# menezesandre/stackrl

Measured on AMD Instinct MI355X. Metric: env steps/sec (batched Stack-v0), higher is better.
Workload: dtype f32

## Files before the change

### stackrl_amd/csrc/settle.hip

```cpp
#include "srl_device.h"
#include "srl_kernels.h"
#include "stage.h"

#ifdef SRL_DIAG_JITTER
__device__ __forceinline__ void srl_jitter_sync() {
  unsigned t = (unsigned)__builtin_readcyclecounter() * 2654435761u + (threadIdx.x >> 6) * 40503u;
  t = __builtin_amdgcn_readfirstlane(t);
  const int n = (t >> 13) & 15;
  for (int i = 0; i < n; ++i) __builtin_amdgcn_s_sleep(16);
  __builtin_amdgcn_fence(__ATOMIC_RELEASE, "workgroup");
  __builtin_amdgcn_s_barrier();
  __builtin_amdgcn_fence(__ATOMIC_ACQUIRE, "workgroup");
  t = t * 1664525u + 1013904223u;
  const int m = (t >> 13) & 15;
  for (int i = 0; i < m; ++i) __builtin_amdgcn_s_sleep(16);
}
#define __syncthreads() srl_jitter_sync()
#endif

#ifndef SRL_GJK_GROUP
#define SRL_GJK_GROUP(T, PP) ((T) == 128 && (PP) == 1 ? 32 : 16)
#endif

__device__ __forceinline__ int pair_word(int p) {
  int j = (int)((1.0f + sqrtf(1.0f + 8.0f * (float)p)) * 0.5f);
  while (j * (j - 1) / 2 > p) --j;
  while ((j + 1) * j / 2 <= p) ++j;
  return (p - j * (j - 1) / 2) | (j << 16);
}

enum { M_MODE = 0, M_U, M_V, M_NEXT, M_ZMAX, M_FLAGS, M_NCOL, M_CNT, M_NB, M_PENDING, M_STATUS, M_DONE, M_ORIENT, M_MOVING, M_RES0, M_RES1, M_SOLO, M_WORDS = 20 };

struct Lds {
  float* sm;
  const DevParams* P;
  int oX, oQ, oV, oPX, oPQ, oMESH, oGM, oMAN, oSOP, oPOS, oCOL, oR, oIW, oAMIN, oAMAX, oBC, oWV, oLV, oMISC, oPAIR, vs3;
  __device__ __forceinline__ void init(float* sm_, const DevParams* P_) {
    sm = sm_; P = P_;
    oX = P->OFF_X; oQ = P->OFF_Q; oV = P->OFF_V; oPX = P->OFF_PX; oPQ = P->OFF_PQ; oMESH = P->OFF_MESH;
    oGM = P->OFF_GM; oMAN = P->OFF_MAN; oSOP = P->OFF_SOP; oPOS = P->OFF_POS; oCOL = P->OFF_COL;
    const int blob = P->BLOB;
    oR = blob + P->S_R; oIW = blob + P->S_IW; oAMIN = blob + P->S_AMIN; oAMAX = blob + P->S_AMAX; oBC = blob + P->S_BC;
    oWV = blob + P->S_WV; oLV = blob + P->S_LV; oMISC = blob + P->S_MISC; oPAIR = blob + P->S_PAIR; vs3 = 3 * P->VS;
#ifndef SRL_NO_LAUNDER
#define SRL_KEEP(x) asm volatile("" : "+s"(x))
    SRL_KEEP(oX); SRL_KEEP(oQ); SRL_KEEP(oV); SRL_KEEP(oPX); SRL_KEEP(oPQ); SRL_KEEP(oMESH); SRL_KEEP(oGM);
    SRL_KEEP(oMAN); SRL_KEEP(oSOP); SRL_KEEP(oPOS); SRL_KEEP(oCOL); SRL_KEEP(oR); SRL_KEEP(oIW); SRL_KEEP(oAMIN);
    SRL_KEEP(oAMAX); SRL_KEEP(oBC); SRL_KEEP(oWV); SRL_KEEP(oLV); SRL_KEEP(oMISC); SRL_KEEP(oPAIR); SRL_KEEP(vs3);
#undef SRL_KEEP
#endif
  }
  __device__ __forceinline__ float* X(int b) const { return sm + oX + 4 * b; }
  __device__ __forceinline__ float* Q(int b) const { return sm + oQ + 4 * b; }
  __device__ __forceinline__ float* VW(int b) const { return sm + oV + 8 * b; }
  __device__ __forceinline__ float* PX(int b) const { return sm + oPX + 4 * b; }
  __device__ __forceinline__ float* PQ(int b) const { return sm + oPQ + 4 * b; }
  __device__ __forceinline__ int* MESH() const { return (int*)(sm + oMESH); }
  __device__ __forceinline__ float* GM(int b) const { return sm + oGM + SRL_GM_WORDS * b; }
  __device__ __forceinline__ float* MAN(int s) const { return sm + oMAN + SRL_MAN_WORDS * s; }
  __device__ __forceinline__ int* SOP() const { return (int*)(sm + oSOP); }
  __device__ __forceinline__ int* POS() const { return (int*)(sm + oPOS); }
  __device__ __forceinline__ int* COL() const { return (int*)(sm + oCOL); }
  __device__ __forceinline__ float* R(int b) const { return sm + oR + 9 * b; }
  __device__ __forceinline__ float* IW(int b) const { return sm + oIW + 9 * b; }
  __device__ __forceinline__ float* AMIN(int b) const { return sm + oAMIN + 3 * b; }
  __device__ __forceinline__ float* AMAX(int b) const { return sm + oAMAX + 3 * b; }
  __device__ __forceinline__ float* BC(int b) const { return sm + oBC + 8 * b; }
  __device__ __forceinline__ float* WV(int b) const { return sm + oWV + vs3 * b; }
  __device__ __forceinline__ float* LV(int b) const { return sm + oLV + vs3 * b; }
  __device__ __forceinline__ int* MISC() const { return (int*)(sm + oMISC); }
  __device__ __forceinline__ int* PAIR() const { return (int*)(sm + oPAIR); }
  __device__ __forceinline__ void pair(int p, int& i, int& j) const { const int w = PAIR()[p]; i = w & 0xffff; j = w >> 16; }
};

typedef float f2 __attribute__((ext_vector_type(2)));
typedef float f4 __attribute__((ext_vector_type(4)));
__device__ __forceinline__ f2 F2(float a, float b) { f2 r; r.x = a; r.y = b; return r; }
__device__ __forceinline__ f2 fma2(f2 a, f2 b, f2 c) { return __builtin_elementwise_fma(a, b, c); }

__device__ __forceinline__ void ldvw(const Lds& L, int b, v3& v, v3& w) {
  const float4 a = *(const float4*)L.VW(b);
  const float2 c = *(const float2*)(L.VW(b) + 4);
  v = V(a.x, a.z, c.x); w = V(a.y, a.w, c.y);
}
__device__ __forceinline__ v3 ldv(const Lds& L, int b) { const float* p = L.VW(b); return V(p[0], p[2], p[4]); }
__device__ __forceinline__ void stvw(const Lds& L, int b, v3 v, v3 w) {
  *(float4*)L.VW(b) = make_float4(v.x, w.x, v.y, w.y);
  *(float2*)(L.VW(b) + 4) = make_float2(v.z, w.z);
}

__device__ void goal_from_rng(const DevParams& P, uint32_t key, uint32_t episode, int32_t* rect) {
  int H = P.c.overhead_res;
  uint32_t bbit = srl_rng(key, episode, SRL_STREAM_GOAL, 0) >> 31;
  uint32_t u0 = srl_rng(key, episode, SRL_STREAM_GOAL, 1) >> 8;
  uint32_t u1 = srl_rng(key, episode, SRL_STREAM_GOAL, 2) >> 8;
  uint32_t u2 = srl_rng(key, episode, SRL_STREAM_GOAL, 3) >> 8;
  uint32_t lo = u0 < u1 ? u0 : u1; lo = lo < u2 ? lo : u2;
  uint32_t hi = u0 > u1 ? u0 : u1; hi = hi > u2 ? hi : u2;
  uint32_t X = bbit ? hi : lo;
  int h = P.goal_min_h + (int)(((uint64_t)X * (uint64_t)(P.goal_max_h - P.goal_min_h)) >> 24);
  int w = P.goal_size / h;
  if (w < P.goal_min_w) w = P.goal_min_w;
  if (w > P.goal_max_w) w = P.goal_max_w;
  int umax = H - h, vmax = H - w;
  int ulo = umax / 8, uhi = 7 * umax / 8 + 1;
  int vlo = vmax / 8, vhi = 7 * vmax / 8 + 1;
  rect[0] = ulo + (int)srl_rng_below(srl_rng(key, episode, SRL_STREAM_GOAL, 4), (uint32_t)(uhi - ulo));
  rect[1] = vlo + (int)srl_rng_below(srl_rng(key, episode, SRL_STREAM_GOAL, 5), (uint32_t)(vhi - vlo));
  rect[2] = h; rect[3] = w;
}

__device__ void env_reset(const DevParams& P, EnvHdr* h, int e) {
  int L = P.c.episode_length;
  uint32_t key = P.seed + (uint32_t)P.c.env_index_offset + (uint32_t)e;
// ... 647 lines not shown
  if (WARM) {
    p.in = p.in * ws; p.i1 = p.i1 * ws; p.i2 = p.i2 * ws;
    prow_apply(p.n, u, p.in);
    prow_apply(p.t1, u, p.i1);
    prow_apply(p.t2, u, p.i2);
  } else {
    prow_solve(p.n, u, p.target, p.in, 0.0f, 1e30f, res);
    const float lim = p.mu * p.in;
    prow_solve(p.t1, u, 0.0f, p.i1, -lim, lim, res);
    prow_solve(p.t2, u, 0.0f, p.i2, -lim, lim, res);
  }
  *(float4*)pa = make_float4(u.a[0].x, u.a[0].y, u.a[1].x, u.a[1].y); *(float2*)(pa + 4) = make_float2(u.a[2].x, u.a[2].y);
  *(float4*)pb = make_float4(u.b[0].x, u.b[0].y, u.b[1].x, u.b[1].y); *(float2*)(pb + 4) = make_float2(u.b[2].x, u.b[2].y);
}

template <bool WARM, int PP, bool SOLO, bool GB, bool GA>
__device__ __forceinline__ bool solver_sweep(const Lds& L, GPoint& gp, GBody& gb, Point (&pp)[PP], int ncol, int gslot,
                                             const int (&pslot)[PP], int gsweep, const unsigned long long (&cm)[2]) {
  float res = 0.0f;
  constexpr unsigned long long T0 = 0x1111111111111111ull;
  if (!GB) {
    const unsigned long long gm = __ballot(gslot >= 0);
#pragma unroll
    for (int i = 0; i < SRL_GMAXP; ++i) {
      const unsigned long long t = gm & (T0 << i);
      if (t == 0) break;
      if (__builtin_amdgcn_inverse_ballot_w64(t)) ground_turn<WARM>(L, gp, res);
      __builtin_amdgcn_wave_barrier();
    }
  } else {
    if (gb.np > 0) ground_body<WARM, !WARM && GA>(L, gb, res);
    __builtin_amdgcn_wave_barrier();
  }
  int c0 = 0;
#ifndef SRL_NO_COLOUR_MASKS
  if (SOLO && PP == 1) {
#pragma unroll
    for (int c = 0; c < 2; ++c) {
      if (c >= ncol) break;
#pragma unroll
      for (int i = 0; i < 4; ++i) {
        const unsigned long long t = cm[c] & (T0 << i);
        if (t == 0) break;
        if (__builtin_amdgcn_inverse_ballot_w64(t)) point_turn<WARM>(L, pp[0], res);
        __builtin_amdgcn_wave_barrier();
      }
    }
    c0 = 2;
  }
#endif
#pragma unroll 1
  for (int c = c0; c < ncol; ++c) {
    if (!SOLO) __syncthreads();
    unsigned long long mc[PP];
#pragma unroll
    for (int r = 0; r < PP; ++r) mc[r] = __ballot((pslot[r] >> 2) == c);
#pragma unroll
    for (int i = 0; i < 4; ++i) {
      unsigned long long any = 0;
#pragma unroll
      for (int r = 0; r < PP; ++r) any |= mc[r] & (T0 << i);
      if (any == 0) break;
#pragma unroll
      for (int r = 0; r < PP; ++r)
        if (__builtin_amdgcn_inverse_ballot_w64(mc[r] & (T0 << i))) point_turn<WARM>(L, pp[r], res);
      __builtin_amdgcn_wave_barrier();
    }
  }
  if (SOLO) return WARM ? true : __ballot(res * res > L.P->c.residual_threshold) != 0ull;
  int* word = L.MISC() + M_RES0 + (gsweep & 1);
  if (!WARM) {
    if (__ballot(res * res > L.P->c.residual_threshold) != 0ull && (threadIdx.x & 63) == 0) *word = gsweep;
  }
  __syncthreads();
  return WARM ? true : *word == gsweep;
}

#ifdef SRL_STAMPS
#define STAMP(k) do { if (tid == 0) { long long _t = wall_clock64(); L.P->hdr[blockIdx.x].stamps[k] += _t - _t0; _t0 = _t; } } while (0)
#else
#define STAMP(k)
#endif

template <int T, int PP>
__device__ __forceinline__ void substep(const Lds& L, int nb, int tid, int& gsweep) {
  const DevParams& P = *L.P;
  if (PP >= 2) asm volatile("" : "+v"(tid));
#ifdef SRL_STAMPS
  long long _t0 = wall_clock64();
#endif
  int* misc = L.MISC();
  if (tid < nb) body_frame(L, tid);
  if (tid == 0) { misc[M_FLAGS] = 0; misc[M_SOLO] = 1; }
  __syncthreads();
  STAMP(0);
  for (int it = tid; it < nb * P.VS; it += T) {
    const int b = it / P.VS, k = it - b * P.VS;
    if (k < __float_as_int(L.BC(b)[5])) {
      const m3 R = ldm(L.R(b));
      v3 lv;
      if (P.S_LV >= 0) lv = ld3(L.LV(b) + 3 * k);
      else { const float4 g4 = P.mv[__float_as_int(L.BC(b)[6]) + k]; lv = V(g4.x, g4.y, g4.z); }
      st3(L.WV(b) + 3 * k, mmul_add(R, lv, ld3(L.X(b))));
    }
  }
  __syncthreads();
  STAMP(1);
  for (int b = tid >> 4; b < nb; b += T >> 4) body_bounds_ground(L, b, tid & 15);
  __syncthreads();
  STAMP(2);
  const int npair = nb * (nb - 1) / 2;
  int fl = 0;
  for (int pid = tid; pid < npair; pid += T) {
    int i, j; L.pair(pid, i, j);
    v3 ai = ld3(L.AMIN(i)), bi = ld3(L.AMAX(i)), aj = ld3(L.AMIN(j)), bj = ld3(L.AMAX(j));
    bool ov = ai.x <= bj.x && aj.x <= bi.x && ai.y <= bj.y && aj.y <= bi.y && ai.z <= bj.z && aj.z <= bi.z;
    int sl = L.SOP()[pid];
    if (!ov && sl >= 0) { L.SOP()[pid] = -1; L.POS()[sl] = -1; fl |= 1; }
    if (ov && sl < 0) fl |= 2;
  }
  if (fl) atomicOr(&misc[M_FLAGS], fl);
  __syncthreads();
  const int flags = misc[M_FLAGS], ncol0 = misc[M_NCOL];
  if (flags || ncol0 < 0) {
    __syncthreads();
    if (tid == 0) {
      if (flags & 2) {
        for (int pid = 0; pid < npair; ++pid) {
          if (L.SOP()[pid] >= 0) continue;
          int i, j; L.pair(pid, i, j);
          v3 ai = ld3(L.AMIN(i)), bi = ld3(L.AMAX(i)), aj = ld3(L.AMIN(j)), bj = ld3(L.AMAX(j));
          bool ov = ai.x <= bj.x && aj.x <= bi.x && ai.y <= bj.y && aj.y <= bi.y && ai.z <= bj.z && aj.z <= bi.z;
          if (!ov) continue;
          int sl = -1;
          for (int k = 0; k < P.NS; ++k) if (L.POS()[k] < 0) { sl = k; break; }
          if (sl < 0) { misc[M_STATUS] |= SRL_ST_PAIR_OVERFLOW; atomicOr(P.flags, 4); continue; }
          L.SOP()[pid] = sl; L.POS()[sl] = pid;
          float* mp = L.MAN(sl);
          mp[0] = __int_as_float(0);
          mp[56] = __int_as_float(0);
          st3(mp + 1, ld3(L.X(i)) - ld3(L.X(j)));
        }
      }
      uint64_t* used = (uint64_t*)(L.sm + P.BLOB + P.S_USED);
      for (int b = 0; b < SRL_MAX_BODIES; ++b) used[b] = 0;
      int nc = 0;
      for (int sl = 0; sl < P.NS; ++sl) {
        int pid = L.POS()[sl];
        if (pid < 0) continue;
        int i, j; L.pair(pid, i, j);
        uint64_t u = used[i] | used[j];
        int c = __ffsll((long long)~u) - 1;
        L.COL()[sl] = c;
        used[i] |= (uint64_t)1 << c;
        used[j] |= (uint64_t)1 << c;
        if (c + 1 > nc) nc = c + 1;
      }
      misc[M_NCOL] = nc;
    }
    __syncthreads();
  }
  const int ncol = misc[M_NCOL];
  STAMP(3);
  {
    constexpr int G = SRL_GJK_GROUP(T, PP);
    const int gl = tid & (G - 1);
    for (int sl = tid / G; sl < P.NS; sl += T / G)
      if (L.POS()[sl] >= 0) narrowphase_slot<G>(L, sl, gl);
  }
  __syncthreads();
  STAMP(4);
  {
    GPoint gp = make_ground_point(L, tid / SRL_GMAXP, tid % SRL_GMAXP);
    if (tid / SRL_GMAXP >= nb) gp.valid = false;
    Point pp[PP];
#pragma unroll
    for (int r = 0; r < PP; ++r) pp[r] = make_pair_point(L, (tid + r * T) >> 2, tid & 3);
    {
      bool mine = gp.valid;
#pragma unroll
      for (int r = 0; r < PP; ++r) mine |= pp[r].valid;
      if (tid >= 64 && __ballot(mine) != 0ull && (tid & 63) == 0) misc[M_SOLO] = 0;
    }
    __syncthreads();
    GBody gb;
    gb.np = 0; gb.b = 0; gb.ima = 0.0f;
    gb.pvw = L.VW(0); gb.rec = cg_rec(L, 0, 0);
#pragma unroll
    for (int i = 0; i < SRL_GMAXP; ++i) { gb.acc[i][0] = 0.0f; gb.acc[i][1] = 0.0f; gb.acc[i][2] = 0.0f; }
#ifdef SRL_GROUND_TURNS
    constexpr bool GB = false;
#else
    constexpr bool GB = !(T == 256 && PP == 1);
#endif
#ifndef SRL_GA_MASK
#define SRL_GA_MASK 1
#endif
    constexpr bool GA = GB && ((T == 128 && PP == 1 && (SRL_GA_MASK & 1)) || (T == 128 && PP == 2 && (SRL_GA_MASK & 2)) ||
                               (T == 256 && PP == 2 && (SRL_GA_MASK & 4)));
    if (GB) {
    if (gp.valid) cg_store(L, gp);
    if (tid < nb) {
      const float* g = L.GM(tid);
      gb.b = tid; gb.np = __float_as_int(g[0]); gb.ima = L.BC(tid)[0];
      gb.pvw = L.VW(tid); gb.rec = cg_rec(L, tid, 0);
#pragma unroll
      for (int i = 0; i < SRL_GMAXP; ++i)
        if (i < gb.np) { gb.acc[i][0] = g[SRL_GM_IN + i]; gb.acc[i][1] = g[SRL_GM_T1 + i]; gb.acc[i][2] = g[SRL_GM_T2 + i]; }
    }
    __syncthreads();
    }
    STAMP(5);
#ifdef SRL_DIAG_NOSOLO
    const bool solo = false;
#else
    const bool solo = PP == 1 && misc[M_SOLO] != 0;
#endif
    const int gslot = gp.valid ? gp.idx : -1;
    unsigned long long cm[2];
    cm[0] = __ballot(pp[0].valid && pp[0].colour == 0); cm[1] = __ballot(pp[0].valid && pp[0].colour == 1);
    int pslot[PP];
#pragma unroll
    for (int r = 0; r < PP; ++r) pslot[r] = pp[r].valid ? 4 * pp[r].colour + pp[r].idx : -1;
    if (solo) {
      int done = 0;
      if (tid < 64) {
        bool anyp = false;
#pragma unroll
        for (int r = 0; r < PP; ++r) anyp |= pp[r].valid;
#ifdef SRL_NO_GROUND_ONLY
        const bool ground_only = false;
#else
        const bool ground_only = GB && __ballot(anyp) == 0ull;
#endif
        if (ground_only) {
          v3 v = V(0.0f, 0.0f, 0.0f), w = V(0.0f, 0.0f, 0.0f);
          if (gb.np > 0) {
            const float4 a0 = *(const float4*)gb.pvw;
            const float2 a1 = *(const float2*)(gb.pvw + 4);
            v = V(a0.x, a0.z, a1.x); w = V(a0.y, a0.w, a1.y);
            float res = 0.0f;
            ground_body_keep<true, false>(L, gb, v, w, res);
          }
          for (int it = 0; it < P.c.solver_iterations; ++it) {
            done++;
            float res = 0.0f;
            if (gb.np > 0) ground_body_keep<false, GA>(L, gb, v, w, res);
            if (__ballot(res * res > P.c.residual_threshold) == 0ull) break;
          }
          if (gb.np > 0) { *(float4*)gb.pvw = make_float4(v.x, w.x, v.y, w.y); *(float2*)(gb.pvw + 4) = make_float2(v.z, w.z); }
        } else {
          solver_sweep<true, PP, PP == 1, GB, GA>(L, gp, gb, pp, ncol, gslot, pslot, 0, cm);
          for (int it = 0; it < P.c.solver_iterations; ++it) {
            done++;
            if (!solver_sweep<false, PP, PP == 1, GB, GA>(L, gp, gb, pp, ncol, gslot, pslot, 0, cm)) break;
          }
        }
        if (tid == 0) misc[M_CNT] = done;
      }
      __syncthreads();
      gsweep += misc[M_CNT];
    } else {
      solver_sweep<true, PP, false, GB, GA>(L, gp, gb, pp, ncol, gslot, pslot, 0, cm);
      for (int it = 0; it < P.c.solver_iterations; ++it) {
        gsweep++;
        if (!solver_sweep<false, PP, false, GB, GA>(L, gp, gb, pp, ncol, gslot, pslot, gsweep, cm)) break;
      }
    }
#ifdef SRL_STAMPS
    if (tid == 0) {
      EnvHdr* hh = &L.P->hdr[blockIdx.x];
      bool anyp = false;
      for (int r = 0; r < PP; ++r) anyp |= pp[r].valid;
      {
        int bl[SRL_MAX_BODIES]; for (int b = 0; b < SRL_MAX_BODIES; ++b) bl[b] = 0;
        int lmax = 0, sumt = 0;
        for (int c = 0; c < ncol; ++c) {
          int mx = 0;
          for (int sl = 0; sl < P.NS; ++sl) {
            const int pid = L.POS()[sl];
            if (pid < 0 || L.COL()[sl] != c) continue;
            const int np = __float_as_int(L.MAN(sl)[0]);
            if (np <= 0) continue;
            int a, b; L.pair(pid, a, b);
            const int st = bl[a] > bl[b] ? bl[a] : bl[b];
            bl[a] = st + np; bl[b] = st + np;
            if (st + np > lmax) lmax = st + np;
            if (np > mx) mx = np;
          }
          sumt += mx;
        }
        hh->diag[4] += sumt; hh->diag[5] += lmax;
      }
      hh->diag[0] += 1; hh->diag[1] += (__ballot(anyp) == 0ull); hh->diag[2] += ncol; hh->diag[3] += solo ? misc[M_CNT] : 0;
    }
#endif
    if (!GB) {
      if (gp.valid) { float* g = L.GM(gp.a); g[SRL_GM_IN + gp.idx] = gp.in; g[SRL_GM_T1 + gp.idx] = gp.i1; g[SRL_GM_T2 + gp.idx] = gp.i2; }
    } else if (gb.np > 0) {
      float* g = L.GM(gb.b);
#pragma unroll
      for (int i = 0; i < SRL_GMAXP; ++i)
        if (i < gb.np) { g[SRL_GM_IN + i] = gb.acc[i][0]; g[SRL_GM_T1 + i] = gb.acc[i][1]; g[SRL_GM_T2 + i] = gb.acc[i][2]; }
    }
#pragma unroll
    for (int r = 0; r < PP; ++r)
      if (pp[r].valid) {
        float* q = L.MAN((tid + r * T) >> 2) + 4 + SRL_MP_WORDS * pp[r].idx;
        q[10] = pp[r].in; q[11] = pp[r].i1; q[12] = pp[r].i2;
      }
  }
  STAMP(6);
  const float dt = P.c.sim_time_step;
  if (tid < nb) {
    const int b = tid;
    v3 v, w;
    ldvw(L, b, v, w);
    st3(L.X(b), madd(ld3(L.X(b)), v, dt));
    float* Q = L.Q(b);
    q4 q; q.x = Q[0]; q.y = Q[1]; q.z = Q[2]; q.w = Q[3];
    float hx = 0.5f * dt;
    q4 dq;
    dq.x = hx * ((w.x * q.w + w.y * q.z) - w.z * q.y);
    dq.y = hx * ((w.y * q.w + w.z * q.x) - w.x * q.z);
    dq.z = hx * ((w.z * q.w + w.x * q.y) - w.y * q.x);
    dq.w = hx * (-((w.x * q.x + w.y * q.y) + w.z * q.z));
    q.x += dq.x; q.y += dq.y; q.z += dq.z; q.w += dq.w;
    float inv = 1.0f / sqrtf((q.x * q.x + q.y * q.y) + (q.z * q.z + q.w * q.w));
    Q[0] = q.x * inv; Q[1] = q.y * inv; Q[2] = q.z * inv; Q[3] = q.w * inv;
  }
  __syncthreads();
  STAMP(7);
}

__device__ __forceinline__ bool sim_stop(const Lds& L, int nb, int tid) {
  int* misc = L.MISC();
  bool moving = false;
  if (tid < nb) {
    v3 v = ldv(L, tid);
    moving = sqrtf(dot(v, v)) > L.P->c.velocity_threshold;
  }
  if (tid < 64) {
    const unsigned long long m = __ballot(moving);
    if (tid == 0) misc[M_MOVING] = m != 0ull;
  }
  __syncthreads();
  const int any = misc[M_MOVING];
  __syncthreads();
  return !any;
}

__device__ __forceinline__ int newest_contacts(const Lds& L, int nb, int tid, int T) {
  int* misc = L.MISC();
  if (tid == 0) misc[M_CNT] = __float_as_int(L.GM(nb - 1)[0]);
  __syncthreads();
  int n = 0;
  for (int sl = tid; sl < L.P->NS; sl += T) {
    int pid = L.POS()[sl];
    int pi_ = -1, pj_ = -1;
    if (pid >= 0) L.pair(pid, pi_, pj_);
    if (pid >= 0 && (pi_ == nb - 1 || pj_ == nb - 1)) n += __float_as_int(L.MAN(sl)[0]);
  }
  if (n) atomicAdd(&misc[M_CNT], n);
  __syncthreads();
  int r = misc[M_CNT];
  __syncthreads();
  return r;
}

__device__ __forceinline__ MeshHdr stage_mesh_hdr(const MeshHdr* __restrict__ mh, int m) {
  MeshHdr r;
  r.vo = __builtin_amdgcn_readfirstlane(mh[m].vo); r.nv = __builtin_amdgcn_readfirstlane(mh[m].nv);
  r.to = __builtin_amdgcn_readfirstlane(mh[m].to); r.nt = __builtin_amdgcn_readfirstlane(mh[m].nt);
  r.eo = __builtin_amdgcn_readfirstlane(mh[m].eo); r.ne = __builtin_amdgcn_readfirstlane(mh[m].ne);
  r.inv_mass = 0.0f; r.iix = 0.0f; r.iiy = 0.0f; r.iiz = 0.0f; r.radius = 0.0f; r.cx = 0.0f; r.cy = 0.0f; r.cz = 0.0f;
  return r;
}

#ifdef SRL_STAGE_TAIL_INLINE
#define SRL_TAIL_ATTR __forceinline__
#else
#define SRL_TAIL_ATTR __attribute__((noinline))
#endif
template <int T>
__device__ SRL_TAIL_ATTR void stage_tail(const DevParams* __restrict__ Pp, float4* __restrict__ stage, int e, int nb) {
  const DevParams& P = *Pp;
  extern __shared__ __attribute__((aligned(16))) float sm[];
  const int tid = threadIdx.x;
  const int wave = __builtin_amdgcn_readfirstlane(tid >> 6), lane = tid & 63;
  StageLds& S = ((StageLds*)(sm + P.BLOB))[wave];
  StageArgs A;
  A.mp = P.mp; A.mt = P.mt; A.me = P.me; A.mv = P.mv; A.px = P.px; A.inv_px = P.inv_px; A.res = P.c.overhead_res;
  const int slots = P.c.episode_length;
  const float* X = sm + P.OFF_X;
  const float* Q = sm + P.OFF_Q;
  const int* MESH = (const int*)(sm + P.OFF_MESH);
  float4* rec0 = stage + (size_t)e * slots * SRL_STAGE_STRIDE;
  int b = wave;
  if (b >= nb) return;
  MeshHdr mh = stage_mesh_hdr(P.mh, __builtin_amdgcn_readfirstlane(MESH[b]));
  StageLoads g = stage_request(A, mh, lane);
  for (;;) {
    const int bn = b + T / 64;
    const bool more = bn < nb;
    MeshHdr mh_n = mh;
    StageLoads g_n = g;
    if (more) { mh_n = stage_mesh_hdr(P.mh, __builtin_amdgcn_readfirstlane(MESH[bn])); g_n = stage_request(A, mh_n, lane); }
    const float* qq = Q + 4 * b;
    q4 q; q.x = qq[0]; q.y = qq[1]; q.z = qq[2]; q.w = qq[3];
    stage_compute(A, S, rec0 + (size_t)b * SRL_STAGE_STRIDE, ld3(X + 4 * b), q, mh, g, lane);
    __builtin_amdgcn_wave_barrier();
    if (!more) break;
// ... 70 lines not shown
        misc[M_RES0] = -1; misc[M_RES1] = -1;
      }
    }
    h->mode = mode;
    misc[M_MODE] = mode;
  }
  __syncthreads();
  const int mode = misc[M_MODE];
  if (mode == 1) {
    int* gi = (int*)gblob;
    for (int k = tid; k < P.NP; k += T) gi[P.OFF_SOP + k] = -1;
    for (int k = tid; k < P.NS; k += T) gi[P.OFF_POS + k] = -1;
    return;
  }
  if (mode == 2 || mode == 3) return;

  for (int k = tid; k < P.BLOB; k += T) sm[k] = gblob[k];
  for (int k = tid; k < P.NP; k += T) L.PAIR()[k] = pair_word(k);
  __syncthreads();

  const int u = misc[M_U], v = misc[M_V], pending = misc[M_PENDING];
  int nb = misc[M_NB];
  if (mode == 0) {
    const int res = P.c.overhead_res, r = P.c.object_res;
    const float* Hm = P.H + (size_t)e * res * res;
    const float* Om = P.objmap + ((size_t)pending * P.n_orient + misc[M_ORIENT]) * r * r;
    uint32_t best = f2o(-1e30f);
    for (int k = tid; k < r * r; k += T) {
      int i = k / r, j = k % r;
      float o = Om[k];
      if (o > 1e-4f) {
        uint32_t s = f2o(Hm[(u + i) * res + (v + j)] + o);
        best = s > best ? s : best;
      }
    }
    atomicMax((uint32_t*)&misc[M_ZMAX], best);
  }
  __syncthreads();
  if (tid == 0 && mode == 0) {
    float z = o2f((uint32_t)misc[M_ZMAX]);
    float half = ((float)P.c.object_res * P.px) * 0.5f;
    v3 pos = V((float)u * P.px + half, (float)v * P.px + half, z - half);
    const MeshHdr mh = P.mh[pending];
    int b = nb;
    L.MESH()[b] = pending;
    if (P.n_orient == 1) {
      st3(L.X(b), P.c.place_at_com ? pos : pos + V(mh.cx, mh.cy, mh.cz));
      L.Q(b)[0] = 0.0f; L.Q(b)[1] = 0.0f; L.Q(b)[2] = 0.0f; L.Q(b)[3] = 1.0f;
    } else {
      const float* oq = P.orient_q[misc[M_ORIENT]];
      q4 q; q.x = oq[0]; q.y = oq[1]; q.z = oq[2]; q.w = oq[3];
      st3(L.X(b), P.c.place_at_com ? pos : pos + mmul(quat_to_mat(q), V(mh.cx, mh.cy, mh.cz)));
      L.Q(b)[0] = q.x; L.Q(b)[1] = q.y; L.Q(b)[2] = q.z; L.Q(b)[3] = q.w;
    }
    stvw(L, b, V(0, 0, 0), V(0, 0, 0));
    L.GM(b)[0] = __int_as_float(0);
  }
  if (mode == 0) nb += 1;
  __syncthreads();
  for (int b = tid; b < nb; b += T) {
    int m = L.MESH()[b];
    const MeshHdr mh = P.mh[m];
    float* bc = L.BC(b);
    bc[0] = mh.inv_mass; bc[1] = mh.iix; bc[2] = mh.iiy; bc[3] = mh.iiz; bc[4] = mh.radius;
    bc[5] = __int_as_float(mh.nv); bc[6] = __int_as_float(mh.vo); bc[7] = __int_as_float(m);
  }
  __syncthreads();
  if (P.S_LV >= 0)
  for (int it = tid; it < nb * P.VS; it += T) {
    const int b = it / P.VS, k = it - b * P.VS;
    const float* bc = L.BC(b);
    if (k < __float_as_int(bc[5])) {
      float4 lv = P.mv[__float_as_int(bc[6]) + k];
      st3(L.LV(b) + 3 * k, V(lv.x, lv.y, lv.z));
    }
  }
  __syncthreads();

  enum { PH_PLACE = 0, PH_SMOOTH = 1, PH_ENTER = 2, PH_SETTLE = 3 };
  int counter = 0, phase = PH_PLACE, s_a = 0;
  int gsweep = 0;
  bool diverged = false;
  if (mode == 4) {
    for (int k = 0; k < -force_reset; ++k) substep<T, PP>(L, nb, tid, gsweep);
    for (int k = tid; k < P.BLOB; k += T) gblob[k] = sm[k];
    if (tid == 0) { h->ncolour = misc[M_NCOL]; h->status = misc[M_STATUS]; h->sweeps = gsweep; }
    return;
  }
  for (;;) {
    if (phase == PH_SMOOTH) {
      if (tid == 0) stvw(L, nb - 1, V(0, 0, 0), V(0, 0, 0));
      __syncthreads();
    }
    substep<T, PP>(L, nb, tid, gsweep);
    counter++;
    if (phase != PH_PLACE && counter > P.max_substeps) diverged = true;
    if (phase == PH_PLACE) phase = P.c.smooth_placing ? PH_SMOOTH : PH_ENTER;
    if (phase == PH_SMOOTH) {
      bool leave = diverged;
      if (!leave) {
        const bool drop = newest_contacts(L, nb, tid, T) >= 3;
        const bool stop = sim_stop(L, nb, tid);
        leave = drop || stop;
      }
      if (leave) phase = PH_ENTER;
    }
    if (phase == PH_ENTER) {
      if (tid == 0 && !diverged) {
        st3(L.PX(nb - 1), ld3(L.X(nb - 1)));
        for (int k = 0; k < 4; ++k) L.PQ(nb - 1)[k] = L.Q(nb - 1)[k];
      }
      s_a = counter;
      phase = PH_SETTLE;
    }
    if (phase == PH_SETTLE && (diverged || sim_stop(L, nb, tid))) break;
  }
  __syncthreads();

  for (int k = tid; k < P.BLOB; k += T) gblob[k] = sm[k];
  if (tid == 0) {
    h->nb = nb;
    h->pending = misc[M_NEXT];
    h->ncolour = misc[M_NCOL];
    h->substeps[0] = s_a;
    h->substeps[1] = counter - s_a;
    h->sweeps = gsweep;
    int st = misc[M_STATUS] | (diverged ? SRL_ST_DIVERGED : 0);
    h->status = st;
    if (diverged) atomicOr(P.flags, 2);
  }

#ifndef SRL_NO_STAGE_TAIL
  if (stage != nullptr) stage_tail<T>(Pp, stage, e, nb);
#endif
}

extern "C" __global__ void __launch_bounds__(128, 2) srl_k_step(const DevParams* __restrict__ Pp,
    const int64_t* __restrict__ action, int force_reset, const int32_t* __restrict__ order, float4* __restrict__ stage) {
  step_body<128, 1>(Pp, action, force_reset, order, stage);
}
extern "C" __global__ void __launch_bounds__(256, 3) srl_k_step_pp1(const DevParams* __restrict__ Pp,
    const int64_t* __restrict__ action, int force_reset, const int32_t* __restrict__ order, float4* __restrict__ stage) {
  step_body<256, 1>(Pp, action, force_reset, order, stage);
}
extern "C" __global__ void __launch_bounds__(256, 2) srl_k_step_pp2(const DevParams* __restrict__ Pp,
    const int64_t* __restrict__ action, int force_reset, const int32_t* __restrict__ order, float4* __restrict__ stage) {
  step_body<256, 2>(Pp, action, force_reset, order, stage);
}

extern "C" __global__ void __launch_bounds__(128, 2) srl_k_step_t128(const DevParams* __restrict__ Pp,
    const int64_t* __restrict__ action, int force_reset, const int32_t* __restrict__ order, float4* __restrict__ stage) {
  step_body<128, 2>(Pp, action, force_reset, order, stage);
}

extern "C" __global__ void __launch_bounds__(64) srl_k_order_keys(const DevParams* __restrict__ Pp,
    const int64_t* __restrict__ action, unsigned long long* __restrict__ keys) {
  const DevParams& P = *Pp;
  const int e = blockIdx.x, lane = threadIdx.x;
  const EnvHdr* h = &P.hdr[e];
  float z = -1.0f;
  int64_t a = action[e];
  if (a != (int64_t)SRL_ACTION_HOLD && !h->done && a >= 0) {
    int slot = 0, mesh = h->pending, nvalid = 1;
    if (P.n_slots > 1) {
      nvalid = P.c.ordering_freedom ? h->list_pos * P.n_orient : P.n_orient;
      slot = (int)(a / (int64_t)P.A);
      a = a % (int64_t)P.A;
      if (P.c.ordering_freedom && slot < nvalid) mesh = h->ids[slot / P.n_orient];
    }
    if (slot < nvalid && a < (int64_t)P.A && mesh >= 0) {
      const int res = P.c.overhead_res, r = P.c.object_res;
      const int u = (int)(a / P.AW), v = (int)(a % P.AW);
      const float* Hm = P.H + (size_t)e * res * res;
      const float* Om = P.objmap + ((size_t)mesh * P.n_orient + slot % P.n_orient) * r * r;
      float best = 0.0f;
      for (int k = lane; k < r * r; k += 64) {
        const float o = Om[k];
        if (o > 1e-4f) best = fmaxf(best, Hm[(u + k / r) * res + (v + k % r)] + o);
      }
      for (int s = 32; s >= 1; s >>= 1) best = fmaxf(best, __shfl_xor(best, s));
      z = best;
    }
  }
  if (lane == 0) keys[e] = ((unsigned long long)(z < 0.0f ? 0xffffffffu : ~__float_as_uint(z)) << 32) | (unsigned)e;
}

extern "C" __global__ void __launch_bounds__(1024) srl_k_order_sort(const unsigned long long* __restrict__ keys, int n, int np2,
                                                                    int32_t* __restrict__ order) {
  extern __shared__ __attribute__((aligned(16))) unsigned long long sk[];
  const int tid = threadIdx.x;
  for (int i = tid; i < np2; i += 1024) sk[i] = i < n ? keys[i] : ~0ull;
  __syncthreads();
  for (int k = 2; k <= np2; k <<= 1)
    for (int j = k >> 1; j >= 1; j >>= 1) {
      for (int t = tid; t < (np2 >> 1); t += 1024) {
        const int i = ((t & ~(j - 1)) << 1) | (t & (j - 1)), p = i | j;
        const unsigned long long a = sk[i], b = sk[p];
        const bool up = (i & k) == 0;
        if ((a > b) == up) { sk[i] = b; sk[p] = a; }
// ... 36 lines not shown
```

### stackrl_amd/csrc/srl_kernels.h

```cpp
#pragma once
#include <stdint.h>
#include "../../include/srl_types.h"

struct MeshHdr {
  int32_t vo, nv, to, nt;
  float inv_mass;
  float iix, iiy, iiz;
  float radius;
  float cx, cy, cz;
  int32_t eo, ne;
};

struct EnvHdr {
  int32_t nb;
  int32_t done;
  uint32_t episode;
  int32_t list_pos;
  int32_t pending;
  int32_t mode;
  int32_t goal[4];
  float prev_metric[4];
  int32_t substeps[2];
  int32_t sweeps;
  int32_t status;
  int32_t ncolour;
  int32_t has_script;
  int32_t ids[SRL_MAX_BODIES];
  int32_t script_ids[SRL_MAX_BODIES];
  int32_t script_goal[4];
#ifdef SRL_STAMPS
  long long stamps[8];
  long long stamps2[4];
  long long rstamps[8];
  long long diag[6];
  long long hwid[2];
#endif
};

struct DevParams {
  srl_config c;
  float px, inv_px, lin_damp, ang_damp, goal_z, scale, elev_num, obj_c1, obj_c2;
  int32_t max_substeps, goal_size, goal_min_h, goal_max_h, goal_min_w, goal_max_w, AW, A;
  int32_t n_mesh, VS , NS , NP ;
  uint32_t seed, sample_counter;
  int32_t force_reset;
  int32_t OFF_X, OFF_Q, OFF_V, OFF_W, OFF_PX, OFF_PQ, OFF_MESH, OFF_GM, OFF_MAN, OFF_SOP, OFF_POS, OFF_COL, BLOB;
  int32_t S_R, S_IW, S_AMIN, S_AMAX, S_BC, S_WV, S_LV, S_USED, S_MISC, S_PAIR, LDS_WORDS;
  EnvHdr* hdr;
  float* blob;
  float* H;
  const MeshHdr* mh;
  const float4* mv;
  const uchar4* mt;
  const uchar4* me;
  const float4* mp;
  const float* objmap;
  int32_t n_orient;
  int32_t n_slots;
  float orient_q[SRL_MAX_ORIENT][4];
  const uint2* codec;
  int32_t codec_n;
  float h_empty;
  uint32_t b_empty, gbyte, zbyte, obj_empty_byte;
  int32_t walk_di, walk_dj;
  uint32_t res_magic;
  const uint8_t* objmap_u8;
  int32_t* flags;
};
```

### stackrl_amd/csrc/stackrl_hip.hip

```cpp
#include <hip/hip_runtime.h>
#include <hip/hip_ext.h>

#include <math.h>
#include <stdio.h>
#include <stdlib.h>
#include <string.h>

#include <vector>

#include "../../include/stackrl_hip.h"
#include "settle.hip"
#include "render.hip"

namespace {

thread_local char g_err[512] = "";

int fail(int code, const char* fmt, const char* arg = "") {
  snprintf(g_err, sizeof g_err, fmt, arg);
  return code;
}

#define HIP_TRY(expr)                                                                    \
  do {                                                                                   \
// ... 645 lines not shown
int srl_get_maps(srl_env* env, float* height, float* object_map, int32_t* goal_rect) {
  if (!env) return fail(SRL_EINVAL, "null env");
  const DevParams& P = env->P;
  const int n = P.c.n_envs, res = P.c.overhead_res, r = P.c.object_res;
  HIP_TRY(hipDeviceSynchronize());
  if (height) HIP_TRY(hipMemcpy(height, P.H, sizeof(float) * (size_t)n * res * res, hipMemcpyDeviceToHost));
  if (object_map || goal_rect) {
    std::vector<EnvHdr> h((size_t)n);
    HIP_TRY(hipMemcpy(h.data(), P.hdr, sizeof(EnvHdr) * (size_t)n, hipMemcpyDeviceToHost));
    for (int i = 0; i < n; ++i) {
      if (goal_rect) for (int k = 0; k < 4; ++k) goal_rect[4 * i + k] = h[i].goal[k];
      if (object_map) {
        const size_t per = (size_t)P.n_orient * r * r;
        const int shown = P.c.ordering_freedom ? P.c.episode_length : 1;
        for (int k = 0; k < shown; ++k) {
          float* o = object_map + ((size_t)i * shown + k) * per;
          const int m = P.c.ordering_freedom ? (k < h[i].list_pos ? h[i].ids[k] : -1) : h[i].pending;
          if (m >= 0) {
            HIP_TRY(hipMemcpy(o, env->d_objmap + (size_t)m * per, sizeof(float) * per, hipMemcpyDeviceToHost));
          } else {
            float e0 = P.obj_c1 - P.obj_c2 / (SRL_FAR + P.c.object_max_dimension * (0.5f - 1.0f));
            for (size_t kk = 0; kk < per; ++kk) o[kk] = e0;
          }
        }
      }
    }
  }
  return SRL_OK;
}

int srl_get_object_map(srl_env* env, int32_t mesh_id, float* object_map) {
  if (!env || !object_map) return fail(SRL_EINVAL, "null argument");
  if (!env->d_objmap) return fail(SRL_ENOMESH, "srl_load_meshes must be called first");
  if (mesh_id < 0 || mesh_id >= env->P.n_mesh) return fail(SRL_EINVAL, "mesh id out of range");
  const size_t per = (size_t)env->P.n_orient * env->P.c.object_res * env->P.c.object_res;
  HIP_TRY(hipMemcpy(object_map, env->d_objmap + (size_t)mesh_id * per, sizeof(float) * per, hipMemcpyDeviceToHost));
  return SRL_OK;
}

int srl_get_stage_records(srl_env* env, float* records, int64_t n_floats) {
  if (!env || !records) return fail(SRL_EINVAL, "null argument");
  const int64_t need = (int64_t)env->P.c.n_envs * env->P.c.episode_length * SRL_STAGE_STRIDE * 4;
  if (n_floats != need) return fail(SRL_EINVAL, "records must hold n_envs x episode_length x SRL_STAGE_STRIDE x 4 floats");
  HIP_TRY(hipDeviceSynchronize());
  HIP_TRY(hipMemcpy(records, env->d_stage, sizeof(float) * (size_t)need, hipMemcpyDeviceToHost));
  return SRL_OK;
}

int32_t srl_stage_record_stride(void) { return SRL_STAGE_STRIDE; }

int srl_render_heightmap(srl_env* env, const float* poses, const int32_t* mesh_ids, const int32_t* n_bodies,
                         float* height, void* stream) {
  if (!env || !poses || !mesh_ids || !n_bodies || !height) return fail(SRL_EINVAL, "null argument");
  if (!env->d_mh) return fail(SRL_ENOMESH, "srl_load_meshes must be called first");
  hipStream_t st = (hipStream_t)stream;
  const int n = env->P.c.n_envs;
  if (!env->d_stage_ext)
    HIP_TRY(hipMalloc((void**)&env->d_stage_ext, sizeof(float4) * (size_t)n * SRL_MAX_BODIES * SRL_STAGE_STRIDE));
  SRL_LAUNCH(env, 2, srl_k_stage, dim3(n, SRL_MAX_BODIES / 4), dim3(256), 0, st, env->P, env->d_stage_ext, SRL_MAX_BODIES, poses,
             mesh_ids, n_bodies);
  SRL_LAUNCH(env, 1, srl_k_render, dim3(n), dim3(SRL_RENDER_THREADS), env->render_lds, st, env->P, (const float4*)env->d_stage_ext,
             SRL_MAX_BODIES, (uint8_t*)nullptr, (uint8_t*)nullptr, (float*)nullptr, (uint8_t*)nullptr, n_bodies, height);
  HIP_TRY(hipGetLastError());
  return SRL_OK;
}

#ifdef SRL_STAMPS
int srl_debug_stamps(srl_env* env, long long* out) {
  const int n = env->P.c.n_envs;
  HIP_TRY(hipDeviceSynchronize());
  std::vector<EnvHdr> h((size_t)n);
  HIP_TRY(hipMemcpy(h.data(), env->P.hdr, sizeof(EnvHdr) * (size_t)n, hipMemcpyDeviceToHost));
  for (int i = 0; i < n; ++i) { for (int k = 0; k < 8; ++k) out[12 * i + k] = h[i].stamps[k]; for (int k = 0; k < 4; ++k) out[12 * i + 8 + k] = h[i].stamps2[k]; }
  return SRL_OK;
}
int srl_debug_hwid(srl_env* env, long long* out) {
  const int n = env->P.c.n_envs;
  HIP_TRY(hipDeviceSynchronize());
  std::vector<EnvHdr> h((size_t)n);
  HIP_TRY(hipMemcpy(h.data(), env->P.hdr, sizeof(EnvHdr) * (size_t)n, hipMemcpyDeviceToHost));
  for (int i = 0; i < n; ++i) { out[2 * i] = h[i].hwid[0]; out[2 * i + 1] = h[i].hwid[1]; }
  return SRL_OK;
}
int srl_debug_diag(srl_env* env, long long* out) {
  const int n = env->P.c.n_envs;
  HIP_TRY(hipDeviceSynchronize());
  std::vector<EnvHdr> h((size_t)n);
  HIP_TRY(hipMemcpy(h.data(), env->P.hdr, sizeof(EnvHdr) * (size_t)n, hipMemcpyDeviceToHost));
  for (int i = 0; i < n; ++i) for (int k = 0; k < 6; ++k) out[6 * i + k] = h[i].diag[k];
  return SRL_OK;
}
int srl_debug_rstamps(srl_env* env, long long* out, int reset) {
  const int n = env->P.c.n_envs;
  HIP_TRY(hipDeviceSynchronize());
  std::vector<EnvHdr> h((size_t)n);
  HIP_TRY(hipMemcpy(h.data(), env->P.hdr, sizeof(EnvHdr) * (size_t)n, hipMemcpyDeviceToHost));
  for (int i = 0; i < n; ++i) for (int k = 0; k < 8; ++k) { out[8 * i + k] = h[i].rstamps[k]; if (reset) h[i].rstamps[k] = 0; }
  if (reset) HIP_TRY(hipMemcpy(env->P.hdr, h.data(), sizeof(EnvHdr) * (size_t)n, hipMemcpyHostToDevice));
  return SRL_OK;
}
#endif

int srl_set_profiling(srl_env* env, int32_t enable) {
  if (!env) return fail(SRL_EINVAL, "null env");
  env->profiling = enable != 0;
  return SRL_OK;
}

int srl_get_kernel_times(srl_env* env, float* ms3, int32_t* launches3) {
  if (!env) return fail(SRL_EINVAL, "null env");
  HIP_TRY(hipDeviceSynchronize());
  for (auto& p : env->pending) {
    float ms = 0.0f;
    if (hipEventElapsedTime(&ms, p.a, p.b) == hipSuccess) { env->acc_ms[p.which] += ms; env->acc_n[p.which] += 1; }
    env->pool.push_back(p.a); env->pool.push_back(p.b);
  }
  env->pending.clear();
  for (int k = 0; k < 3; ++k) {
    if (ms3) ms3[k] = env->acc_ms[k];
    if (launches3) launches3[k] = env->acc_n[k];
    env->acc_ms[k] = 0.0f; env->acc_n[k] = 0;
  }
  return SRL_OK;
}

int srl_get_order_kernel_times(srl_env* env, float* ms, int32_t* launches) {
  if (!env) return fail(SRL_EINVAL, "null env");
  if (!env->pending.empty()) return fail(SRL_EINVAL, "call srl_get_kernel_times first (it collects the pending events)");
  if (ms) *ms = env->acc_ms[3];
  if (launches) *launches = env->acc_n[3];
  env->acc_ms[3] = 0.0f; env->acc_n[3] = 0;
  return SRL_OK;
}

int srl_get_launch_order(srl_env* env, unsigned long long* keys, int32_t* order) {
  if (!env || !keys || !order) return fail(SRL_EINVAL, "null argument");
  if (!env->d_order) return fail(SRL_EINVAL, "this handle has no launch-order buffers (more than 16,384 envs)");
  const int n = env->P.c.n_envs;
  HIP_TRY(hipDeviceSynchronize());
  HIP_TRY(hipMemcpy(keys, env->d_order_keys, sizeof(unsigned long long) * (size_t)n, hipMemcpyDeviceToHost));
  HIP_TRY(hipMemcpy(order, env->d_order, sizeof(int32_t) * (size_t)n, hipMemcpyDeviceToHost));
  return SRL_OK;
}

}
```

Measured before the change: 99520.

## Fuse stop/contact checks into substep, compact live narrowphase slots, move ground points to wave 1

The integration tail of each substep now computes the per-body moving flag and the newest body's contact count with a single wave ballot and shuffle reduction. It stores both in shared misc words so the outer loop no longer calls sim_stop and newest_contacts, which carry their own barriers. For the 128-thread PP=1 variant, narrowphase work is assigned by compacting live slots from a ballot mask instead of striding over all slots. Ground points are also built only on wave 1, which frees wave 0 and removes it from the solo check. The changes add a branchy slot-assignment loop and a slightly longer integration tail, and they depend on NS fitting in 64 lanes.

After: 100,100 (median of 5 runs). No clear change (+0.6%).

```diff
diff --git a/stackrl_amd/csrc/settle.hip b/stackrl_amd/csrc/settle.hip
--- a/stackrl_amd/csrc/settle.hip
+++ b/stackrl_amd/csrc/settle.hip
@@ -29,7 +29,7 @@
   return (p - j * (j - 1) / 2) | (j << 16);
 }
 
-enum { M_MODE = 0, M_U, M_V, M_NEXT, M_ZMAX, M_FLAGS, M_NCOL, M_CNT, M_NB, M_PENDING, M_STATUS, M_DONE, M_ORIENT, M_MOVING, M_RES0, M_RES1, M_SOLO, M_WORDS = 20 };
+enum { M_MODE = 0, M_U, M_V, M_NEXT, M_ZMAX, M_FLAGS, M_NCOL, M_CNT, M_NB, M_PENDING, M_STATUS, M_DONE, M_ORIENT, M_MOVING, M_RES0, M_RES1, M_SOLO, M_NEWC, M_WORDS = 20 };
 
 struct Lds {
   float* sm;
@@ -843,8 +843,24 @@
 #define STAMP(k)
 #endif
 
+#ifdef SRL_NO_FUSED_STOP
+#define SRL_FUSED_STOP 0
+#else
+#define SRL_FUSED_STOP 1
+#endif
+#ifdef SRL_NO_GROUND_WAVE1
+#define SRL_GROUND_WAVE1(T, PP) false
+#else
+#define SRL_GROUND_WAVE1(T, PP) ((T) == 128 && (PP) == 1)
+#endif
+#ifdef SRL_NO_LIVE_SLOTS
+#define SRL_LIVE_SLOTS(T, PP) false
+#else
+#define SRL_LIVE_SLOTS(T, PP) ((T) == 128 && (PP) == 1)
+#endif
+
 template <int T, int PP>
-__device__ __forceinline__ void substep(const Lds& L, int nb, int tid, int& gsweep) {
+__device__ __forceinline__ void substep(const Lds& L, int nb, int tid, int& gsweep, bool want_contacts) {
   const DevParams& P = *L.P;
   if (PP >= 2) asm volatile("" : "+v"(tid));
 #ifdef SRL_STAMPS
@@ -926,19 +942,71 @@
   {
     constexpr int G = SRL_GJK_GROUP(T, PP);
     const int gl = tid & (G - 1);
+#ifdef SRL_STAMPS
+    if (tid == 0) {
+      int cnt[T / G], live = 0, mx = 0;
+      for (int g = 0; g < T / G; ++g) cnt[g] = 0;
+      for (int sl = 0; sl < P.NS; ++sl) if (L.POS()[sl] >= 0) { live++; cnt[sl % (T / G)]++; }
+      for (int g = 0; g < T / G; ++g) mx = cnt[g] > mx ? cnt[g] : mx;
+      EnvHdr* hh = &L.P->hdr[blockIdx.x];
+      if (SRL_LIVE_SLOTS(T, PP)) mx = (live + T / G - 1) / (T / G);
+      hh->stamps3[2] += mx; hh->stamps3[3] += live; hh->stamps3[4] += live > 0;
+    }
+#endif
+    if constexpr (SRL_LIVE_SLOTS(T, PP)) {
+      const int lane = tid & 63, grp = tid / G;
+      unsigned long long m = __ballot(lane < P.NS && L.POS()[lane < P.NS ? lane : 0] >= 0);
+      while (m != 0ull) {
+        int sl = -1;
+#pragma unroll
+        for (int k = 0; k < T / G; ++k) {
+          const int s = m != 0ull ? (int)__builtin_ctzll(m) : -1;
+          m &= m - 1ull;
+          sl = grp == k ? s : sl;
+        }
+        if (sl >= 0) {
+#ifdef SRL_STAMPS
+          const long long _p0 = wall_clock64();
+#endif
+          narrowphase_slot<G>(L, sl, gl);
+#ifdef SRL_STAMPS
+          if (tid == 0) L.P->hdr[blockIdx.x].stamps3[1] += wall_clock64() - _p0;
+#endif
+        }
+      }
+    } else
     for (int sl = tid / G; sl < P.NS; sl += T / G)
-      if (L.POS()[sl] >= 0) narrowphase_slot<G>(L, sl, gl);
+      if (L.POS()[sl] >= 0) {
+#ifdef SRL_STAMPS
+        const long long _p0 = wall_clock64();
+#endif
+        narrowphase_slot<G>(L, sl, gl);
+#ifdef SRL_STAMPS
+        if (tid == 0) L.P->hdr[blockIdx.x].stamps3[1] += wall_clock64() - _p0;
+#endif
+      }
   }
   __syncthreads();
   STAMP(4);
   {
-    GPoint gp = make_ground_point(L, tid / SRL_GMAXP, tid % SRL_GMAXP);
-    if (tid / SRL_GMAXP >= nb) gp.valid = false;
+#ifdef SRL_GROUND_TURNS
+    constexpr bool GB = false;
+#else
+    constexpr bool GB = !(T == 256 && PP == 1);
+#endif
+    constexpr bool GW = GB && SRL_GROUND_WAVE1(T, PP);
+    static_assert(!GW || (T == 128 && PP == 1), "GW: the variant of <= 8 rocks, whose 32 ground points fit wave 1's lanes");
+    const int gt = GW ? tid - 64 : tid;
+    GPoint gp = {};
+    if (!GW || tid >= 64) {
+      gp = make_ground_point(L, gt / SRL_GMAXP, gt % SRL_GMAXP);
+      if (gt / SRL_GMAXP >= nb) gp.valid = false;
+    }
     Point pp[PP];
 #pragma unroll
     for (int r = 0; r < PP; ++r) pp[r] = make_pair_point(L, (tid + r * T) >> 2, tid & 3);
     {
-      bool mine = gp.valid;
+      bool mine = GW ? false : gp.valid;
 #pragma unroll
       for (int r = 0; r < PP; ++r) mine |= pp[r].valid;
       if (tid >= 64 && __ballot(mine) != 0ull && (tid & 63) == 0) misc[M_SOLO] = 0;
@@ -949,11 +1017,6 @@
     gb.pvw = L.VW(0); gb.rec = cg_rec(L, 0, 0);
 #pragma unroll
     for (int i = 0; i < SRL_GMAXP; ++i) { gb.acc[i][0] = 0.0f; gb.acc[i][1] = 0.0f; gb.acc[i][2] = 0.0f; }
-#ifdef SRL_GROUND_TURNS
-    constexpr bool GB = false;
-#else
-    constexpr bool GB = !(T == 256 && PP == 1);
-#endif
 #ifndef SRL_GA_MASK
 #define SRL_GA_MASK 1
 #endif
@@ -1073,10 +1136,12 @@
   }
   STAMP(6);
   const float dt = P.c.sim_time_step;
+  bool moving = false;
   if (tid < nb) {
     const int b = tid;
     v3 v, w;
     ldvw(L, b, v, w);
+    if (SRL_FUSED_STOP) moving = sqrtf(dot(v, v)) > P.c.velocity_threshold;
     st3(L.X(b), madd(ld3(L.X(b)), v, dt));
     float* Q = L.Q(b);
     q4 q; q.x = Q[0]; q.y = Q[1]; q.z = Q[2]; q.w = Q[3];
@@ -1089,6 +1154,24 @@
     q.x += dq.x; q.y += dq.y; q.z += dq.z; q.w += dq.w;
     float inv = 1.0f / sqrtf((q.x * q.x + q.y * q.y) + (q.z * q.z + q.w * q.w));
     Q[0] = q.x * inv; Q[1] = q.y * inv; Q[2] = q.z * inv; Q[3] = q.w * inv;
+  }
+  if (SRL_FUSED_STOP && tid < 64) {
+    const unsigned long long mv = __ballot(moving);
+    int n = 0;
+    if (want_contacts) {
+      for (int sl = tid; sl < P.NS; sl += 64) {
+        const int pid = L.POS()[sl];
+        int pi_ = -1, pj_ = -1;
+        if (pid >= 0) L.pair(pid, pi_, pj_);
+        if (pid >= 0 && (pi_ == nb - 1 || pj_ == nb - 1)) n += __float_as_int(L.MAN(sl)[0]);
+      }
+#pragma unroll
+      for (int sh = 32; sh >= 1; sh >>= 1) n += __shfl_xor(n, sh);
+    }
+    if (tid == 0) {
+      misc[M_MOVING] = mv != 0ull;
+      if (want_contacts) misc[M_NEWC] = n + __float_as_int(L.GM(nb - 1)[0]);
+    }
   }
   __syncthreads();
   STAMP(7);
@@ -1325,25 +1408,40 @@
   int gsweep = 0;
   bool diverged = false;
   if (mode == 4) {
-    for (int k = 0; k < -force_reset; ++k) substep<T, PP>(L, nb, tid, gsweep);
+    for (int k = 0; k < -force_reset; ++k) substep<T, PP>(L, nb, tid, gsweep, false);
     for (int k = tid; k < P.BLOB; k += T) gblob[k] = sm[k];
     if (tid == 0) { h->ncolour = misc[M_NCOL]; h->status = misc[M_STATUS]; h->sweeps = gsweep; }
     return;
   }
+#ifdef SRL_STAMPS
+  long long _tb = wall_clock64();
+#define STAMP_BETWEEN() do { if (tid == 0) P.hdr[blockIdx.x].stamps3[0] += wall_clock64() - _tb; } while (0)
+#else
+#define STAMP_BETWEEN()
+#endif
   for (;;) {
     if (phase == PH_SMOOTH) {
       if (tid == 0) stvw(L, nb - 1, V(0, 0, 0), V(0, 0, 0));
       __syncthreads();
     }
-    substep<T, PP>(L, nb, tid, gsweep);
+    if (counter) STAMP_BETWEEN();
+    substep<T, PP>(L, nb, tid, gsweep, phase != PH_SETTLE);
+#ifdef SRL_STAMPS
+    _tb = wall_clock64();
+#endif
     counter++;
     if (phase != PH_PLACE && counter > P.max_substeps) diverged = true;
     if (phase == PH_PLACE) phase = P.c.smooth_placing ? PH_SMOOTH : PH_ENTER;
     if (phase == PH_SMOOTH) {
       bool leave = diverged;
       if (!leave) {
+#if SRL_FUSED_STOP
+        const bool drop = misc[M_NEWC] >= 3;
+        const bool stop = !misc[M_MOVING];
+#else
         const bool drop = newest_contacts(L, nb, tid, T) >= 3;
         const bool stop = sim_stop(L, nb, tid);
+#endif
         leave = drop || stop;
       }
       if (leave) phase = PH_ENTER;
@@ -1356,8 +1454,13 @@
       s_a = counter;
       phase = PH_SETTLE;
     }
+#if SRL_FUSED_STOP
+    if (phase == PH_SETTLE && (diverged || !misc[M_MOVING])) break;
+#else
     if (phase == PH_SETTLE && (diverged || sim_stop(L, nb, tid))) break;
-  }
+#endif
+  }
+  STAMP_BETWEEN();
   __syncthreads();
 
   for (int k = tid; k < P.BLOB; k += T) gblob[k] = sm[k];
diff --git a/stackrl_amd/csrc/srl_kernels.h b/stackrl_amd/csrc/srl_kernels.h
--- a/stackrl_amd/csrc/srl_kernels.h
+++ b/stackrl_amd/csrc/srl_kernels.h
@@ -33,6 +33,7 @@
   long long stamps2[4];
   long long rstamps[8];
   long long diag[6];
+  long long stamps3[6];
   long long hwid[2];
 #endif
 };
diff --git a/stackrl_amd/csrc/stackrl_hip.hip b/stackrl_amd/csrc/stackrl_hip.hip
--- a/stackrl_amd/csrc/stackrl_hip.hip
+++ b/stackrl_amd/csrc/stackrl_hip.hip
@@ -751,6 +751,14 @@
   for (int i = 0; i < n; ++i) { out[2 * i] = h[i].hwid[0]; out[2 * i + 1] = h[i].hwid[1]; }
   return SRL_OK;
 }
+int srl_debug_stamps3(srl_env* env, long long* out) {
+  const int n = env->P.c.n_envs;
+  HIP_TRY(hipDeviceSynchronize());
+  std::vector<EnvHdr> h((size_t)n);
+  HIP_TRY(hipMemcpy(h.data(), env->P.hdr, sizeof(EnvHdr) * (size_t)n, hipMemcpyDeviceToHost));
+  for (int i = 0; i < n; ++i) for (int k = 0; k < 6; ++k) out[6 * i + k] = h[i].stamps3[k];
+  return SRL_OK;
+}
 int srl_debug_diag(srl_env* env, long long* out) {
   const int n = env->P.c.n_envs;
   HIP_TRY(hipDeviceSynchronize());
```
